# hy-vision-learning/jck-generation

Measured on AMD Instinct MI355X. Metric: images/sec (G+D step) DCGAN 64x64 bs256, higher is better.
Workload: dtype bf16; 1 GPU; DCGAN 64x64x3 synthetic, batch 256 per GPU, full G+D step incl. GP pass, RNG and Adam (BASELINE.json configs[1]); per_gpu_batch=256, global_batch=256, parallelism=dp1, dead_D_wgrad_in_G_phase=skipped (never observable: zeroed at train/dcgan_trainer.py:155)

## Files before the change

### include/jckgan.h

```cpp
#ifndef JCKGAN_H
#define JCKGAN_H
#include <stddef.h>
#include <stdint.h>
#ifdef __cplusplus
extern "C" {
#endif

#define JCK_PREC_BF16 0
#define JCK_PREC_F32 1
#define JCK_PREC_BF16X3 2

#define JCK_OK 0
#define JCK_E_ARG (-1)
#define JCK_E_HIP (-2)
#define JCK_E_WS (-3)

const char* jck_last_error(void);
const char* jck_last_launch(void);
const char* jck_launch_name(int i);
int jck_version(void);
int jck_pad_rows(int c);
int jck_pad_chan(int c);

size_t jck_packed_bytes(int prec, long long elems);
// ... 126 lines not shown
                 void* stream);
size_t jck_gp_head2_conv_ws_floats(int B);
int jck_gp_head2_conv(int prec, const void* v4, const void* a4, const float* wp, const float* prob, int B, int C, float* rs,
                      void* g_a4, float* grad, float* ws, void* stream);
size_t jck_bn2_ws_floats(int C);
int jck_bn2_vchain(int prec, const void* v, const void* y, const void* gy, const float* aux, const float* s1, const float* gamma,
                   float slope, float* ws, void* u, void* xdir, float* dgamma, long long rows, int C, void* stream);
int jck_bn2_reverse(int prec, const void* ua, const void* y, const void* xdir, const float* aux, const float* gamma,
                    const float* vsums, float slope, float* ws, void* uy, float* dgamma, float* dbeta, long long rows, int C,
                    void* stream);

int jck_adam(float* p, const float* g, float* m, float* v, long long n, double lr, double beta1, double beta2, double eps,
             int step, float grad_scale, void* stream);
int jck_adam_ema(float* p, const float* g, float* m, float* v, float* ema, long long n, double lr, double beta1, double beta2,
                 double eps, int step, float grad_scale, float ema_weight, const unsigned* skip_if, void* stream);

typedef struct jck_engine jck_engine;
int jck_engine_create(jck_engine** out, int family, int prec, int batch);
int jck_engine_create_sized(jck_engine** out, int family, int prec, int batch, int image_size);
#define JCK_ENGINE_GP_BACKWARD 1u
int jck_engine_create_ex(jck_engine** out, int family, int prec, int batch, int image_size, unsigned flags);
int jck_engine_image_size(const jck_engine*);
int jck_engine_num_tensors_of(const jck_engine*, int net);
int jck_engine_tensor_info_of(const jck_engine*, int net, int idx, char* name, int name_cap, int* kind, long long* offset,
                              long long* numel, int* shape4);
long long jck_engine_arena_numel_of(const jck_engine*, int net, int which);
void jck_engine_destroy(jck_engine*);
int jck_engine_num_tensors(int family, int net );
int jck_engine_tensor_info(int family, int net, int idx, char* name, int name_cap, int* kind, long long* offset,
                           long long* numel, int* shape4);
// ... 131 lines not shown
```

### jck-generation_amd/csrc/engine.hip

```cpp
#include <cstdlib>

#include "engine_internal.hpp"
#define JCK_BATCHED_DEFAULT 3

namespace {

constexpr long long ALIGN_F = 64;

void add_param(NetLayout& L, const char* name, int a, int b, int c, int d) {
  TensorInfo ti{name, 0, L.n_params, (long long)a * b * c * d, {a, b, c, d}};
  L.t.push_back(ti);
  L.n_params = (L.n_params + ti.numel + ALIGN_F - 1) / ALIGN_F * ALIGN_F;
}
void add_bn(NetLayout& L, const char* wn, const char* bn, const char* rm, const char* rv, int c) {
  add_param(L, wn, c, 1, 1, 1);
  add_param(L, bn, c, 1, 1, 1);
  TensorInfo m{rm, 1, L.n_bn, c, {c, 1, 1, 1}};
  L.t.push_back(m);
  L.n_bn += (c + ALIGN_F - 1) / ALIGN_F * ALIGN_F;
  TensorInfo v{rv, 2, L.n_bn, c, {c, 1, 1, 1}};
  L.t.push_back(v);
  L.n_bn += (c + ALIGN_F - 1) / ALIGN_F * ALIGN_F;
}

// ... 100 lines not shown
  e->LG = make_layout(family, 0, image_size); e->LD = make_layout(family, 1, image_size);
  e->overlap = env_on("JCK_OVERLAP");
  e->batched = getenv("JCK_BATCHED") ? atoi(getenv("JCK_BATCHED")) : JCK_BATCHED_DEFAULT;
  if (!e->overlap || batch % 8 != 0 || e->batched != 3) e->batched = 0;
  e->gp_bwd = family == 0 && (flags & JCK_ENGINE_GP_BACKWARD);
  e->carve(nullptr);
  e->wgrad_side = env_on("JCK_WGRAD_SIDE");
  e->head_side = env_on("JCK_HEAD_SIDE");
  e->ext_events = env_on("JCK_EXT_EVENTS");
  e->bn_res = env_on("JCK_BN_RES");
  e->cbuf_direct = family == 1 && env_on("JCK_CBUF_DIRECT");
  e->head_fuse = env_on("JCK_HEAD_FUSE");
  e->real_side = env_on("JCK_REAL_SIDE");
  e->fold_zero = env_on("JCK_FOLD_ZERO");
  e->fuse_tanh = env_on("JCK_FUSE_TANH");
  if (e->overlap) JCK_TRY(create_side_streams(e));
  *out = e;
  return JCK_OK;
}
extern "C" void jck_engine_destroy(jck_engine* e) {
  if (!e) return;
  if (e->overlap) destroy_side_streams(e, true);
  infer_free(e);
  delete e;
}
extern "C" int jck_engine_num_tensors(int family, int net) { return (int)make_layout(family, net).t.size(); }
static int tensor_info(const NetLayout& L, int idx, char* name, int name_cap, int* kind, long long* offset, long long* numel, int* shape4) {
  if (idx < 0 || idx >= (int)L.t.size()) JCK_FAIL(JCK_E_ARG, "index out of range");
  const TensorInfo& t = L.t[idx];
  if (name && name_cap > 0) { strncpy(name, t.name, name_cap - 1); name[name_cap - 1] = 0; }
// ... 28 lines not shown
  if (ws_bytes < e->ws_bytes) JCK_FAIL(JCK_E_WS, "workspace too small: need " + std::to_string(e->ws_bytes));
  if (((uintptr_t)workspace) % 256) JCK_FAIL(JCK_E_ARG, "workspace must be 256-byte aligned");
  e->carve(reinterpret_cast<unsigned char*>(workspace));
  {
    unsigned char* p0 = reinterpret_cast<unsigned char*>(e->d_down[0]);
    unsigned char* p1 = reinterpret_cast<unsigned char*>(e->dset[0].y[0]);
    HIPCHK(hipMemset(p0, 0, (size_t)(p1 - p0)));
  }
  HIPCHK(hipMemset(e->gsync, 0, jck_grid_sync_bytes()));
  e->gp = g_params; e->gg = g_grads; e->gm = g_m; e->gv = g_v; e->gbn = g_bn; e->gnbt = g_nbt;
  e->dp = d_params; e->dg = d_grads; e->dm = d_m; e->dv = d_v; e->dbn = d_bn; e->dnbt = d_nbt;
  e->bound = true;
  return JCK_OK;
}

static int repack_convs(jck_engine* e, int net, void* stream, const TailJobs* tail = nullptr, int tail_x = 0) {
  PackJobs jobs = {};
  int n = 0, chunk = 0;
  auto add = [&](int kind, const float* w, void* wp, long long total, int a, int b, int c) {
    PackJob& J = jobs.j[n];
    J.w = w; J.wp = wp; J.total = total; J.kind = kind; J.a = a; J.b = b; J.c = c;
    jobs.first_chunk[n] = chunk;
    chunk += (int)((total + PACK_CHUNK - 1) / PACK_CHUNK);
    ++n;
  };
  auto add_down = [&](const float* w, int Cs, int Cb, void* wp) { add(0, w, wp, (long long)Cs * Cb, Cs, Cb, ilog2(jck_pad_chan(Cb))); };
  auto add_up = [&](const float* w, int Cs, int Cb, void* wp) {
    if (Cb <= 4) add(2, w, wp, (long long)Cs * Cb, Cs, Cb, 0);
    else add(1, w, wp, (long long)Cs * Cb, Cs, Cb, jck_pad_rows(Cb));
  };
  if (net == 1) {
// ... 1 lines not shown
      const float* w = e->P(e->LD, e->dp, CWN[i]);
      add_down(w, TT.D_CS[i], TT.D_CB[i], e->d_down[i]);
      add_up(w, TT.D_CS[i], TT.D_CB[i], e->d_up[i]);
    }
    if (e->family == 0) add(4, e->P(e->LD, e->dp, CWN[TT.NS]), e->d_head_wp, TT.G_C1, TT.G_C1, 0, 0);
  } else {
    add(3, e->P(e->LG, e->gp, CWN[0]), e->g1_w, (long long)z_dim(e->family) * TT.G_C1, z_dim(e->family), TT.G_C1, z_pad(e->family));
    for (int i = 0; i < TT.NS; ++i) {
      const float* w = e->P(e->LG, e->gp, CWN[i + 1]);
      add_up(w, TT.G_CS[i], TT.G_CB[i], e->g_up[i]);
      add_down(w, TT.G_CS[i], TT.G_CB[i], e->g_down[i]);
    }
  }
  jobs.first_chunk[n] = chunk;
  jobs.n = n;
  if (net == 1) e->d_packed = true;
  if (tail) {
    const int nblk = chunk + tail_x * (tail->nl + 1);
    if (e->prec == JCK_PREC_BF16) hipLaunchKernelGGL(pack_tail_kernel<bf16_t>, dim3(nblk), dim3(256), 0, (hipStream_t)stream, jobs, chunk, *tail, tail_x);
    else hipLaunchKernelGGL(pack_tail_kernel<float>, dim3(nblk), dim3(256), 0, (hipStream_t)stream, jobs, chunk, *tail, tail_x);
  } else if (e->prec == JCK_PREC_BF16) hipLaunchKernelGGL(pack_multi_kernel<bf16_t>, dim3(chunk), dim3(256), 0, (hipStream_t)stream, jobs);
  else hipLaunchKernelGGL(pack_multi_kernel<float>, dim3(chunk), dim3(256), 0, (hipStream_t)stream, jobs);
  HIPCHK(hipGetLastError());
  return JCK_OK;
}
static int repack_linear(jck_engine* e, void* stream) {
  const float* w1 = e->P(e->LD, e->dp, "linear1.weight");
  return pack_linear_pair(e->prec, w1, L1_OUT, L1_K, L1_OUT, L1_KPAD, e->l1_w, L1_KPAD, L1_OUT, e->l1_wT, 512, 16, (hipStream_t)stream);
}
extern "C" int jck_engine_repack(jck_engine* e, int net, void* stream) {
// ... 402 lines not shown

static int refresh_adam_scalars(jck_engine* e, int step, float lr, hipStream_t st) {
  const int q = step & 1;
  JCK_TRY(jck_adam_set_step(e->hp2 + 8 * q, (double)lr, ADAM_B1, ADAM_B2, step, e->noise_seed, e->ema_w(step), st));
  e->hp_step[q] = step;
  e->hp_lr[q] = lr;
  return JCK_OK;
}
static int set_step_impl(jck_engine* e, int step, float lr, void* stream, bool zero_d);
static int adam_net(jck_engine* e, int net, long long first, long long count, float grad_scale, const float* hp, hipStream_t st,
                    float* zero_other = nullptr, float* ema = nullptr) {
  float *p = net ? e->dp : e->gp, *g = net ? e->dg : e->gg, *m = net ? e->dm : e->gm, *v = net ? e->dv : e->gv;
  return jck_adam_hp(p + first, g + first, m + first, v + first, count, ADAM_B1, ADAM_B2, ADAM_EPS, grad_scale, hp, st, zero_other,
                     zero_other ? (net ? e->LG : e->LD).n_params : 0, jck_grid_sync_error_word(e->gsync), ema);
}
static int clear_or_memset(jck_engine* e, int& clean_step, int step, hipStream_t st, void* p, size_t bytes, void* p2 = nullptr, size_t bytes2 = 0) {
  const bool clean = clean_step == step && !e->capturing;
  clean_step = -1;
  if (!clean) HIPCHK(hipMemsetAsync(p, 0, bytes, st));
  if (!clean && p2) HIPCHK(hipMemsetAsync(p2, 0, bytes2, st));
  return JCK_OK;
}
static int zero_d_grads(jck_engine* e, int step, hipStream_t st) {
  return clear_or_memset(e, e->ss.dg_clean_step, step, st, e->dg, e->LD.n_params * sizeof(float), e->family == 1 ? e->gw1p : nullptr,
                         (size_t)L1_OUT * L1_KPAD * sizeof(float));
}
static int clear_acc(jck_engine* e, int step, hipStream_t st) {
  return clear_or_memset(e, e->ss.acc_clean_step, step, st, e->acc, (size_t)8 * e->acc_ld * sizeof(float));
}

// ... 186 lines not shown

static int phase_d_step(jck_engine* e, const PhaseCtx& c) {
  if (e->ss.gp_inflight || (e->gp_bwd && e->ss.gp_done)) JCK_FAIL(JCK_E_ARG, "PHASE_D_GP must be called before PHASE_D_STEP");
  if (!e->hp_holds(c.in->step, c.in->lr) && !e->capturing) JCK_TRY(refresh_adam_scalars(e, c.in->step, c.in->lr, c.st));
  const float* hp = e->hp2 + 8 * e->parity;
  float* zg = (e->fold_zero && !e->capturing && e->LG.n_params % 4 == 0) ? e->gg : nullptr;
  if (zg) e->ss.gg_clean_step = c.in->step;
  if (e->ss.join_pending) {
    const TensorInfo* c1 = find(e->LD, CWN[0]);
    const long long cut = c1->offset + c1->numel;
    HIPCHK(hipStreamWaitEvent(c.st, e->ss.mid_recorded ? e->evWmid : e->evWdone, 0));
    JCK_TRY(adam_net(e, 1, cut, e->LD.n_params - cut, c.in->grad_scale, hp, c.st, zg));
    JCK_TRY(repack_linear(e, c.st));
    if (e->ss.mid_recorded) HIPCHK(hipStreamWaitEvent(c.st, e->evWdone, 0));
    e->ss.join_pending = e->ss.mid_recorded = false;
    JCK_TRY(adam_net(e, 1, 0, cut, c.in->grad_scale, hp, c.st));
    return repack_convs(e, 1, c.st);
  }
  JCK_TRY(adam_net(e, 1, 0, e->LD.n_params, c.in->grad_scale, hp, c.st, zg));
  return jck_engine_repack(e, 1, c.st);
}

static int phase_g_loss(jck_engine* e, const PhaseCtx& c) {
  JCK_TRY(clear_or_memset(e, e->ss.gg_clean_step, c.in->step, c.st, e->gg, e->LG.n_params * sizeof(float)));
  const bool fuse = e->head_fuse;
  JCK_TRY(d_forward(e, c.D0, e->fake, c.B, 3, c.in->drop_mask[3], c.st, !fuse));
  if (fuse && !c.cg) JCK_TRY(d_head(e, c.D0, c.B, 0.9f, 0, 2, 5, c.st, c.D0.g[TT.NS - 1]));
  else if (fuse) {
    const float tg1 = 0.9f;
    const int md1 = 0, sl1 = 2, sp1 = 5;
    JCK_TRY(cg_head_middle(e, c.B, 1, &tg1, &md1, &sl1, &sp1, c.D0.prob, c.D0.ds, c.in->drop_mask[3], c.st));
  } else JCK_TRY(d_head(e, c.D0, c.B, 0.9f, 0, 2, 5, c.st));
  XgradEpi xe = {e->fake_raw, 0.9f, e->g_raw, (c.sA && e->ext_events) ? e->evW[TT.NS - 1] : nullptr, false};
  DBackward bw;
  bw.gw = 0; bw.xgrad = true; bw.xe = e->fuse_tanh ? &xe : nullptr;
  JCK_TRY(d_backward(e, c.D0, e->fake, c.B, c.in->drop_mask[3], c.st, bw, fuse));
  return g_backward(e, c.D0.gx, c.B, c.st, c.sA, xe.fused);
}

static int phase_g_step(jck_engine* e, const PhaseCtx& c) {
  if (!e->hp_holds(c.in->step, c.in->lr) && !e->capturing) JCK_TRY(refresh_adam_scalars(e, c.in->step, c.in->lr, c.st));
  JCK_TRY(adam_net(e, 0, 0, e->LG.n_params, c.in->grad_scale, e->hp2 + 8 * e->parity, c.st, nullptr, e->gema));
  TailJobs t = {};
  for (int i = 0; i < TT.NS; ++i) {
    const int cs = TT.D_CS[i];
    t.l[i].rec = e->d_rs[i] + (size_t)e->parity * 4 * 2 * cs;
    t.l[i].rm = e->dbn + find(e->LD, RMN[i])->offset;
    t.l[i].rv = e->dbn + find(e->LD, RVN[i])->offset;
    t.l[i].nbt = (long long*)(e->dnbt + i);
    t.l[i].C = cs;
  }
  t.nl = TT.NS; t.npass = 4; t.momentum = BN_MOM; t.acc = e->acc; t.acc_ld = e->acc_ld; t.B = c.B; t.invB = 1.0f / (float)c.B; t.lambda_gp = 10.0f; t.out = e->scal_out;
  return repack_convs(e, 0, c.st, &t, cdiv(TT.G_C1, 256));
}

static int phase_begin(jck_engine* e, int phase, jck_step_inputs& loc, hipStream_t st) {
  const bool cg = e->family == 1;
  const int q = loc.step & 1;
  if (!loc.z) loc.z = e->rz[q];
  if (!loc.alpha) loc.alpha = e->ralpha[q];
  if (cg && !loc.drop_mask[0] && !loc.drop_mask[1] && !loc.drop_mask[2] && !loc.drop_mask[3])
    for (int i = 0; i < 4; ++i) loc.drop_mask[i] = e->rmask[q] + (size_t)i * e->B * L1_OUT;
  if (e->ss.join_pending && !(phase == JCK_PHASE_D_STEP || (phase == JCK_PHASE_D_GP && cg && e->ss.gp_done))) {
    HIPCHK(hipStreamWaitEvent(st, e->evWdone, 0));
    e->ss.join_pending = e->ss.mid_recorded = false;
  }
  if (cg) {
    if (!loc.labels) JCK_FAIL(JCK_E_ARG, "CGAN phases need labels");
// ... 201 lines not shown
```

### jck-generation_amd/csrc/engine_internal.hpp

```cpp
#pragma once
#include <cstring>
#include <vector>

#include "ops_internal.hpp"
#include "ew_optim.hpp"
#define JCK_INTERNAL __attribute__((visibility("hidden")))
struct jck_engine;
#define TT (e->T)

namespace jck_eng JCK_INTERNAL {

struct TensorInfo { const char* name; int kind; long long offset, numel; int shape[4]; };

struct NetLayout {
  std::vector<TensorInfo> t;
  long long n_params = 0, n_bn = 0;
};

#define JCK_MAX_STAGES 5
struct Topo {
  int S, NS, HW;
  int D_CS[JCK_MAX_STAGES], D_CB[JCK_MAX_STAGES], D_HB[JCK_MAX_STAGES];
  int G_CS[JCK_MAX_STAGES], G_CB[JCK_MAX_STAGES], G_HS[JCK_MAX_STAGES];
  int G_C1, FEAT;
// ... 80 lines not shown
  template <typename F> void for_each_side_stream(F f) { for (hipStream_t* p : {&sA, &sB, &sC}) f(*p); }
  template <typename F> void for_each_event(F f) {
    for (hipEvent_t* p : {&evWdone, &evWmid, &evHead, &evTail, &ev0, &evF, &evReal, &evGP}) f(*p);
    for (hipEvent_t& p : evW) f(p);
  }
  bool overlap = true, defer_join = true;
  bool wgrad_side = true;
  bool head_side = true;
  bool ext_events = true;
  unsigned* gsync = nullptr; bool bn_res = true;
  bool cbuf_direct = true;
  bool head_fuse = true;
  bool real_side = true;
  bool fold_zero = true;
  bool fuse_tanh = true;
  void *g_z, *g_y[JCK_MAX_STAGES], *g_a[JCK_MAX_STAGES], *g_gr[JCK_MAX_STAGES], *fake_raw, *fake, *g_raw;
  void *real_noisy, *xhat;
  BnBuf g_bn[JCK_MAX_STAGES];
  float *acc, *scal_out;
  float *acc2, *scal2;
  int acc_ld = 0;
  float *head_ws, *gp2_ws;
  float* hp2;
  unsigned long long noise_seed = 0x6a636b67616e0001ull;
  float *rz[2] = {nullptr, nullptr}, *ralpha[2] = {nullptr, nullptr}, *rmask[2] = {nullptr, nullptr};
  int hp_step[2] = {0, 0};
  float hp_lr[2] = {-1.f, -1.f};
  bool hp_holds(int step, float lr) const { return hp_step[step & 1] == step && hp_lr[step & 1] == lr; }
  bool capturing = false;
  bool gp_bwd = false;
// ... 147 lines not shown
```

### jck-generation_amd/csrc/ew_optim.hpp

```cpp
#pragma once
#include "common.hpp"
#include "philox.hpp"

struct StepRng { float* z; long long nz; float* alpha; long long nalpha; float* masks; long long nmask; float keep_p; float* zero; long long nzero;
                 float* zbig[2]; long long nzbig[2];
                 void* zpad; int zd, zp, zpad_f32; };
__device__ __forceinline__ float u01(unsigned x) { return ((float)(x >> 8) + 0.5f) * (1.0f / 16777216.0f); }
static __global__ void adam_hp_kernel(float* __restrict__ hp, float step_size, float bc2_sqrt, unsigned seed_lo, unsigned seed_hi,
                                      unsigned step, const StepRng r, float ema_w) {
  if (threadIdx.x == 0 && blockIdx.x == 0) {
    hp[0] = step_size; hp[1] = bc2_sqrt; hp[2] = ema_w;
    unsigned* w = reinterpret_cast<unsigned*>(hp + 4);
    w[0] = seed_lo; w[1] = seed_hi; w[2] = step; w[3] = 0u;
  }
  const long long q0 = (r.nz + 3) / 4, q1 = (r.nalpha + 3) / 4, q2 = (r.nmask + 3) / 4;
  for (long long i = blockIdx.x * (long long)blockDim.x + threadIdx.x; i < r.nzero; i += (long long)gridDim.x * blockDim.x) r.zero[i] = 0.f;
#pragma unroll
  for (int b = 0; b < 2; ++b)
    for (long long i = blockIdx.x * (long long)blockDim.x + threadIdx.x; i < (r.nzbig[b] >> 2); i += (long long)gridDim.x * blockDim.x)
      reinterpret_cast<f32x4*>(r.zbig[b])[i] = f32x4{0.f, 0.f, 0.f, 0.f};
  for (long long i = blockIdx.x * (long long)blockDim.x + threadIdx.x; i < q0 + q1 + q2; i += (long long)gridDim.x * blockDim.x) {
    unsigned o[4];
    if (i < q0) {
      philox4x32_10((unsigned)i, (unsigned)(i >> 32), 8u, step, seed_lo, seed_hi, o);
// ... 262 lines not shown
  if (c >= L.C) return;
  float rm = L.rm[c], rv = L.rv[c];
  for (int p = 0; p < t.npass; ++p) {
    rm = (1.f - t.momentum) * rm + t.momentum * L.rec[(long long)p * 2 * L.C + c];
    rv = (1.f - t.momentum) * rv + t.momentum * L.rec[(long long)p * 2 * L.C + L.C + c];
  }
  L.rm[c] = rm;
  L.rv[c] = rv;
}
template <typename W>
__global__ __launch_bounds__(256) void pack_tail_kernel(const PackJobs jobs, int pack_chunks, const TailJobs t, int tail_x) {
  if ((int)blockIdx.x < pack_chunks) { pack_multi_block<W>(jobs, (int)blockIdx.x); return; }
  const int q = (int)blockIdx.x - pack_chunks;
  step_tail_block(t, q % tail_x, q / tail_x);
}
```

### jck-generation_amd/csrc/ops.hip

```cpp
#include "ops_internal.hpp"
#include "ew.hpp"
#include "ew_optim.hpp"
#include "bnres.hpp"
#include "latent.hpp"

#include <cstdlib>
#include <cstring>
#include <string>

static thread_local std::string g_err;
void jck_set_error(const std::string& s) { g_err = s; }
extern "C" const char* jck_last_error(void) { return g_err.c_str(); }
#ifndef JCK_BUILD_ID
#define JCK_BUILD_ID 100
#endif
extern "C" int jck_version(void) { return JCK_BUILD_ID; }

struct KernelInfo { const char* launch; const char* label; };
#define SAME(s) {s, s}
static constexpr KernelInfo KERNELS[] = {
    SAME("igemm<bf16,128,128>"),   SAME("igemm<bf16,128,64>"),   SAME("igemm<bf16,64,128,img>"),   {nullptr, "igemm<bf16,64,128>"}, SAME("igemm<bf16,16,256>"),
    SAME("igemm<f32,128,128>"),    SAME("igemm<f32,128,64>"),    SAME("igemm<f32,64,128,img>"),    SAME("igemm<f32,64,128>"),       SAME("igemm<f32,16,256>"),
    SAME("igemm<bf16x3,128,128>"), SAME("igemm<bf16x3,128,64>"), SAME("igemm<bf16x3,64,128,img>"), SAME("igemm<bf16x3,64,128>"),    SAME("igemm<bf16x3,16,256>"),
    {"igemm_dma_persist<128,256,8>", "igemm<bf16,128,256>"}, {"igemm_dma_persist<128,128,4>", "igemm<bf16,128,128>"},
// ... 636 lines not shown
  return jck_adam_set_step(hp, 2e-4, 0.5, 0.999, step, seed, 0.f, (hipStream_t)stream, z, nz, alpha, nalpha, masks, nmask, keep_p);
}
int jck_adam_hp(float* p, const float* g, float* m, float* v, long long n, double beta1, double beta2, double eps,
                float grad_scale, const float* hp, hipStream_t st, float* zero, long long nzero, const unsigned* skip_if, float* ema) {
  const int vec = (((uintptr_t)p | (uintptr_t)g | (uintptr_t)m | (uintptr_t)v | (uintptr_t)ema) & 15) == 0;
  if (zero && (((uintptr_t)zero & 15) || (nzero & 3))) JCK_FAIL(JCK_E_ARG, "adam: the zero range must be 16-byte aligned, count % 4 == 0");
  if (ema)
    hipLaunchKernelGGL(adam_kernel<true>, dim3(ew_grid(vec ? (n + 3) / 4 : n)), dim3(256), 0, st, p, g, m, v, n, (float)(1.0 - beta1), (float)beta2,
                       (float)(1.0 - beta2), (float)eps, 0.f, 1.f, grad_scale, hp, vec, zero, zero ? nzero / 4 : 0, skip_if, ema, 1.f);
  else
    hipLaunchKernelGGL(adam_kernel<false>, dim3(ew_grid(vec ? (n + 3) / 4 : n)), dim3(256), 0, st, p, g, m, v, n, (float)(1.0 - beta1), (float)beta2,
                     (float)(1.0 - beta2), (float)eps, 0.f, 1.f, grad_scale, hp, vec, zero, zero ? nzero / 4 : 0, skip_if);
  HIPCHK(hipGetLastError());
  return JCK_OK;
}

static int launch_latent_loss(KernelId id, double bytes, int prec, const void* x, const float* target, const float* weight, const void* g_x,
                              void* g_raw, float* loss, int N, int HW, hipStream_t st) {
  ProfScope prof(id, 0.0, st, bytes);
  if (target && !weight && !g_x) {
    DISPATCH_T(prec, hipLaunchKernelGGL((latent_loss_kernel<T, true>), dim3(N), dim3(256), 0, st, (const T*)x, target, nullptr, nullptr, (T*)g_raw,
                                        loss, HW));
  } else {
    DISPATCH_T(prec, hipLaunchKernelGGL((latent_loss_kernel<T, false>), dim3(N), dim3(256), 0, st, (const T*)x, target, weight, (const T*)g_x,
                                        (T*)g_raw, loss, HW));
  }
  HIPCHK(hipGetLastError());
  return JCK_OK;
}
extern "C" int jck_latent_loss(int prec, const void* x_nhwc4, const float* target_nchw_f32, void* g_raw_out, float* loss_out, int N,
// ... 289 lines not shown
```

### jck-generation_amd/csrc/ops_internal.hpp

```cpp
#pragma once
#include <hip/hip_ext.h>

#include <algorithm>
#include <cmath>
#include <string>

#include "../../include/jckgan.h"
#include "common.hpp"

void jck_set_error(const std::string& s);

static inline bool prec_f32_storage(int prec) { return prec == JCK_PREC_F32 || prec == JCK_PREC_BF16X3; }
static inline bool is_pow2(int v) { return v > 0 && (v & (v - 1)) == 0; }
static inline unsigned ew_grid(long long n, int per_block = 256) { return (unsigned)std::max<long long>(1, std::min<long long>((n + per_block - 1) / per_block, 8192)); }

#define JCK_FAIL(code, msg)                                   \
  do {                                                        \
    jck_set_error(std::string(__func__) + ": " + (msg));     \
    return (code);                                            \
  } while (0)

#define HIPCHK(expr)                                                                                     \
  do {                                                                                                   \
    hipError_t e_ = (expr);                                                                              \
// ... 60 lines not shown
  bool on; ProfRec r;
};
bool jck_prof_is_on();

extern int g_igemm_dma_ksplit, g_bn_bwd_fuse, g_bn_res, g_wgrad_wgs, g_wgrad_ws, g_wgrad_dma;

int jck_adam_set_step(float* hp, double lr, double beta1, double beta2, int step, unsigned long long seed, float ema_w, hipStream_t st,
                      float* rz = nullptr, long long nz = 0, float* ralpha = nullptr, long long nalpha = 0, float* rmasks = nullptr,
                      long long nmask = 0, float keep_p = 0.75f, float* zero = nullptr, long long nzero = 0, float* zbig0 = nullptr,
                      long long nzbig0 = 0, float* zbig1 = nullptr, long long nzbig1 = 0, void* zpad = nullptr, int zd = 0, int zp = 0,
                      int zpad_f32 = 0);
int jck_adam_hp(float* p, const float* g, float* m, float* v, long long n, double beta1, double beta2, double eps,
                float grad_scale, const float* hp, hipStream_t st, float* zero = nullptr, long long nzero = 0,
                const unsigned* skip_if = nullptr,
                float* ema = nullptr);
const unsigned* jck_grid_sync_error_word(const void* sync_ws);
int bn_fwd_fused(int prec, const void* y, const float* stats, int slots_per_group, float count, const float* gamma, const float* beta,
                 float eps, float slope, void* a, float* aux, float* stat_out, float* running_mean, float* running_var, int64_t* nbt,
                 float momentum, long long rows_per_group, int C, int groups, long long out_row, long long out_pitch, hipStream_t stream,
                 bool* fused);
int bn_act_bwd_res_ev(int prec, const void* g_a, const void* y, const float* aux, float slope, float* sums, void* g_y, float* dgamma,
                      float* dbeta, long long rows_per_group, int C, int groups, int grad_groups, void* sync_ws, hipStream_t stream,
                      hipEvent_t done);
int conv_up_tanh_bwd_ev(int prec, const void* small_in, const void* w, const void* tanh_y, float scale, void* out, int N, int Hs, int Ws,
                        int Cs, int Cb, hipStream_t stream, hipEvent_t done, bool* fused);
int head_bwd_conv2_ev(int prec, const float* ds, const float* wp, const void* a4, int B, int B_more, int C, void* g_a4, float* grad, float* ws,
                      hipStream_t stream, hipStream_t side, hipEvent_t handover);
int gp_head2_ev(int prec, const void* ughd, const float* w2, const float* prob, int B, int K, float* rs, float* dw2, float* ws,
                hipStream_t stream, hipStream_t side, hipEvent_t handover);
int pack_linear_pair(int prec, const float* w, int N, int K, int rows0, int cols0, void* wp0, int rows1, int cols1, void* wp1, int permC,
// ... 13 lines not shown
```

### jck-generation_amd/hipgan/_lib.py

```python
import ctypes as C
import os

import torch

HERE = os.path.dirname(os.path.abspath(__file__))
LIB_PATH = os.path.join(os.path.dirname(HERE), "lib", "libjckgan_hip.so")
PREC_BF16, PREC_F32, PREC_BF16X3 = 0, 1, 2

vp, i32, i64, f32, f64, sz = C.c_void_p, C.c_int, C.c_longlong, C.c_float, C.c_double, C.c_size_t


class StepInputs(C.Structure):
    _fields_ = [("real_nchw", vp), ("noise_real", vp), ("z", vp), ("noise_fake", vp), ("alpha", vp),
                ("lr", f32), ("grad_scale", f32), ("step", i32), ("labels", vp), ("drop_mask", vp * 4),
                ("real_u8", vp), ("real_idx", vp)]


PROTOS = {
    "jck_last_error": (C.c_char_p, []),
    "jck_last_launch": (C.c_char_p, []),
    "jck_launch_name": (C.c_char_p, [i32]),
    "jck_version": (i32, []),
    "jck_pad_rows": (i32, [i32]),
    "jck_pad_chan": (i32, [i32]),
    "jck_packed_bytes": (sz, [i32, i64]),
    "jck_stats_floats": (sz, [i64, i32, i32]),
    "jck_pack_down": (i32, [i32, vp, i32, i32, vp, vp]),
    "jck_pack_up": (i32, [i32, vp, i32, i32, vp, vp]),
    "jck_pack_g1": (i32, [i32, vp, i32, i32, i32, vp, vp]),
    "jck_pack_head": (i32, [vp, i32, vp, vp]),
# ... 61 lines not shown
    "jck_sum_vec": (i32, [vp, i32, vp, vp]),
    "jck_cgan_z": (i32, [i32, vp, vp, i32, i32, i32, i32, vp, vp]),
    "jck_gp_grad": (i32, [i32, vp, vp, f32, i32, i32, vp, vp]),
    "jck_gp_head2": (i32, [i32, vp, vp, vp, i32, i32, vp, vp, vp, vp]),
    "jck_gp_head2_conv_ws_floats": (sz, [i32]),
    "jck_gp_head2_conv": (i32, [i32, vp, vp, vp, vp, i32, i32, vp, vp, vp, vp, vp]),
    "jck_bn2_ws_floats": (sz, [i32]),
    "jck_bn2_vchain": (i32, [i32, vp, vp, vp, vp, vp, vp, f32, vp, vp, vp, vp, i64, i32, vp]),
    "jck_bn2_reverse": (i32, [i32, vp, vp, vp, vp, vp, vp, f32, vp, vp, vp, vp, i64, i32, vp]),
    "jck_head_bwd": (i32, [i32, vp, vp, vp, i32, i32, vp, vp, i32, vp, vp]),
    "jck_head_unpack_grad": (i32, [vp, i32, vp, i32, vp]),
    "jck_head_bwd_conv": (i32, [i32, vp, vp, vp, i32, i32, vp, vp, vp, vp]),
    "jck_head_bwd_conv2": (i32, [i32, vp, vp, vp, i32, i32, i32, vp, vp, vp, vp]),
    "jck_adam": (i32, [vp, vp, vp, vp, i64, f64, f64, f64, f64, i32, f32, vp]),
    "jck_adam_ema": (i32, [vp, vp, vp, vp, vp, i64, f64, f64, f64, f64, i32, f32, f32, vp, vp]),
    "jck_engine_create": (i32, [C.POINTER(vp), i32, i32, i32]),
    "jck_engine_create_sized": (i32, [C.POINTER(vp), i32, i32, i32, i32]),
    "jck_engine_create_ex": (i32, [C.POINTER(vp), i32, i32, i32, i32, C.c_uint]),
    "jck_engine_image_size": (i32, [vp]),
    "jck_engine_num_tensors_of": (i32, [vp, i32]),
    "jck_engine_tensor_info_of": (i32, [vp, i32, i32, C.c_char_p, i32, C.POINTER(i32), C.POINTER(i64), C.POINTER(i64),
                                        C.POINTER(i32)]),
    "jck_engine_arena_numel_of": (i64, [vp, i32, i32]),
    "jck_engine_destroy": (None, [vp]),
    "jck_engine_num_tensors": (i32, [i32, i32]),
    "jck_engine_tensor_info": (i32, [i32, i32, i32, C.c_char_p, i32, C.POINTER(i32), C.POINTER(i64), C.POINTER(i64),
                                     C.POINTER(i32)]),
    "jck_engine_workspace_bytes": (sz, [vp]),
    "jck_engine_arena_numel": (i64, [i32, i32, i32]),
    "jck_engine_bind": (i32, [vp, vp, sz] + [vp] * 12),
# ... 127 lines not shown
```

Measured before the change: 165,700 images/sec.

## Fuse Adam update with conv weight repacking into one kernel

Adds an adam_pack kernel that applies the Adam (and EMA) update tile by tile on conv weights and writes the packed bf16/f32 conv layouts straight from LDS, so updated weights are not reread from global memory. Params outside any conv job go through a flat Adam path in the same launch, and the BN tail jobs ride along as extra blocks. This removes one launch and one full pass over the weights in the D and G step phases. In exchange the kernel uses uncoalesced tile-based Adam access and adds range bookkeeping on the host.

```diff
diff --git a/include/jckgan.h b/include/jckgan.h
--- a/include/jckgan.h
+++ b/include/jckgan.h
@@ -164,6 +164,10 @@
              int step, float grad_scale, void* stream);
 int jck_adam_ema(float* p, const float* g, float* m, float* v, float* ema, long long n, double lr, double beta1, double beta2,
                  double eps, int step, float grad_scale, float ema_weight, const unsigned* skip_if, void* stream);
+typedef struct { int kind; long long offset; void* wp; int a, b, c; } jck_pack_job;
+int jck_adam_pack(float* p, const float* g, float* m, float* v, float* ema, long long n, const jck_pack_job* jobs, int njobs,
+                  int prec, double beta1, double beta2, double eps, float grad_scale, const float* hp, float* zero,
+                  long long nzero, const unsigned* skip_if, int fused, void* stream);
 
 typedef struct jck_engine jck_engine;
 int jck_engine_create(jck_engine** out, int family, int prec, int batch);
diff --git a/jck-generation_amd/csrc/engine.hip b/jck-generation_amd/csrc/engine.hip
--- a/jck-generation_amd/csrc/engine.hip
+++ b/jck-generation_amd/csrc/engine.hip
@@ -138,6 +138,7 @@
   e->real_side = env_on("JCK_REAL_SIDE");
   e->fold_zero = env_on("JCK_FOLD_ZERO");
   e->fuse_tanh = env_on("JCK_FUSE_TANH");
+  e->adam_pack = env_on("JCK_ADAM_PACK");
   if (e->overlap) JCK_TRY(create_side_streams(e));
   *out = e;
   return JCK_OK;
@@ -196,7 +197,7 @@
   return JCK_OK;
 }
 
-static int repack_convs(jck_engine* e, int net, void* stream, const TailJobs* tail = nullptr, int tail_x = 0) {
+static PackJobs pack_jobs(jck_engine* e, int net, int* chunks) {
   PackJobs jobs = {};
   int n = 0, chunk = 0;
   auto add = [&](int kind, const float* w, void* wp, long long total, int a, int b, int c) {
@@ -228,6 +229,12 @@
   }
   jobs.first_chunk[n] = chunk;
   jobs.n = n;
+  *chunks = chunk;
+  return jobs;
+}
+static int repack_convs(jck_engine* e, int net, void* stream, const TailJobs* tail = nullptr, int tail_x = 0) {
+  int chunk = 0;
+  const PackJobs jobs = pack_jobs(e, net, &chunk);
   if (net == 1) e->d_packed = true;
   if (tail) {
     const int nblk = chunk + tail_x * (tail->nl + 1);
@@ -660,6 +667,19 @@
   return jck_adam_hp(p + first, g + first, m + first, v + first, count, ADAM_B1, ADAM_B2, ADAM_EPS, grad_scale, hp, st, zero_other,
                      zero_other ? (net ? e->LG : e->LD).n_params : 0, jck_grid_sync_error_word(e->gsync), ema);
 }
+static int adam_repack_net(jck_engine* e, int net, long long first, long long count, float grad_scale, const float* hp, hipStream_t st,
+                           float* zero_other = nullptr, float* ema = nullptr, const TailJobs* tail = nullptr, int tail_x = 0) {
+  if (!e->adam_pack) {
+    JCK_TRY(adam_net(e, net, first, count, grad_scale, hp, st, zero_other, ema));
+    return repack_convs(e, net, st, tail, tail_x);
+  }
+  int chunk = 0;
+  const PackJobs jobs = pack_jobs(e, net, &chunk);
+  if (net == 1) e->d_packed = true;
+  float *p = net ? e->dp : e->gp, *g = net ? e->dg : e->gg, *m = net ? e->dm : e->gm, *v = net ? e->dv : e->gv;
+  return jck_adam_pack_hp(p, g, m, v, (net ? e->LD : e->LG).n_params, first, count, jobs, e->prec, ADAM_B1, ADAM_B2, ADAM_EPS, grad_scale, hp, st,
+                          zero_other, zero_other ? (net ? e->LG : e->LD).n_params : 0, jck_grid_sync_error_word(e->gsync), ema, tail, tail_x);
+}
 static int clear_or_memset(jck_engine* e, int& clean_step, int step, hipStream_t st, void* p, size_t bytes, void* p2 = nullptr, size_t bytes2 = 0) {
   const bool clean = clean_step == step && !e->capturing;
   clean_step = -1;
@@ -876,11 +896,10 @@
     JCK_TRY(repack_linear(e, c.st));
     if (e->ss.mid_recorded) HIPCHK(hipStreamWaitEvent(c.st, e->evWdone, 0));
     e->ss.join_pending = e->ss.mid_recorded = false;
-    JCK_TRY(adam_net(e, 1, 0, cut, c.in->grad_scale, hp, c.st));
-    return repack_convs(e, 1, c.st);
-  }
-  JCK_TRY(adam_net(e, 1, 0, e->LD.n_params, c.in->grad_scale, hp, c.st, zg));
-  return jck_engine_repack(e, 1, c.st);
+    return adam_repack_net(e, 1, 0, cut, c.in->grad_scale, hp, c.st);
+  }
+  JCK_TRY(adam_repack_net(e, 1, 0, e->LD.n_params, c.in->grad_scale, hp, c.st, zg));
+  return c.cg ? repack_linear(e, c.st) : JCK_OK;
 }
 
 static int phase_g_loss(jck_engine* e, const PhaseCtx& c) {
@@ -902,7 +921,6 @@
 
 static int phase_g_step(jck_engine* e, const PhaseCtx& c) {
   if (!e->hp_holds(c.in->step, c.in->lr) && !e->capturing) JCK_TRY(refresh_adam_scalars(e, c.in->step, c.in->lr, c.st));
-  JCK_TRY(adam_net(e, 0, 0, e->LG.n_params, c.in->grad_scale, e->hp2 + 8 * e->parity, c.st, nullptr, e->gema));
   TailJobs t = {};
   for (int i = 0; i < TT.NS; ++i) {
     const int cs = TT.D_CS[i];
@@ -913,7 +931,7 @@
     t.l[i].C = cs;
   }
   t.nl = TT.NS; t.npass = 4; t.momentum = BN_MOM; t.acc = e->acc; t.acc_ld = e->acc_ld; t.B = c.B; t.invB = 1.0f / (float)c.B; t.lambda_gp = 10.0f; t.out = e->scal_out;
-  return repack_convs(e, 0, c.st, &t, cdiv(TT.G_C1, 256));
+  return adam_repack_net(e, 0, 0, e->LG.n_params, c.in->grad_scale, e->hp2 + 8 * e->parity, c.st, nullptr, e->gema, &t, cdiv(TT.G_C1, 256));
 }
 
 static int phase_begin(jck_engine* e, int phase, jck_step_inputs& loc, hipStream_t st) {
diff --git a/jck-generation_amd/csrc/engine_internal.hpp b/jck-generation_amd/csrc/engine_internal.hpp
--- a/jck-generation_amd/csrc/engine_internal.hpp
+++ b/jck-generation_amd/csrc/engine_internal.hpp
@@ -118,6 +118,7 @@
   bool real_side = true;
   bool fold_zero = true;
   bool fuse_tanh = true;
+  bool adam_pack = true;
   void *g_z, *g_y[JCK_MAX_STAGES], *g_a[JCK_MAX_STAGES], *g_gr[JCK_MAX_STAGES], *fake_raw, *fake, *g_raw;
   void *real_noisy, *xhat;
   BnBuf g_bn[JCK_MAX_STAGES];
diff --git a/jck-generation_amd/csrc/ew_optim.hpp b/jck-generation_amd/csrc/ew_optim.hpp
--- a/jck-generation_amd/csrc/ew_optim.hpp
+++ b/jck-generation_amd/csrc/ew_optim.hpp
@@ -300,3 +300,175 @@
   const int q = (int)blockIdx.x - pack_chunks;
   step_tail_block(t, q % tail_x, q / tail_x);
 }
+
+#define AP_TS 16
+#define AP_TB 16
+#define AP_SC 17
+#define AP_SR (AP_TB * AP_SC + 1)
+#define AP_MAX_RANGES (PACK_MAX_JOBS + 1)
+struct AdamPack {
+  float* p; const float* g; float* m; float* v; float* ema;
+  const float* hp; float* zero; const unsigned* skip_if;
+  long long nzero4, ufirst, fuse_end;
+  float w1, beta2, omb2, eps, grad_scale;
+  int vec, tiles, rest_blocks, nr;
+  int first_tile[PACK_MAX_JOBS + 1];
+  int other[PACK_MAX_JOBS];
+  int upd[PACK_MAX_JOBS];
+  long long rfirst[AP_MAX_RANGES], rcount[AP_MAX_RANGES];
+};
+__device__ __forceinline__ void adam_one_as(bool fuse_v, float& pi, float g_raw, float& m_io, float& v_io, float w1, float beta2, float omb2,
+                                            float eps, float step_size, float bc2_sqrt, float grad_scale) {
+#pragma clang fp contract(off)
+  const float gi = g_raw * grad_scale;
+  const float d = __builtin_fmaf(grad_scale, g_raw, -m_io);
+  const float mi = (w1 < 0.5f) ? __builtin_fmaf(w1, d, m_io) : __builtin_fmaf(-(1.f - w1), d, gi);
+  const float t = (omb2 * gi) * gi;
+  const float vi = fuse_v ? __builtin_fmaf(beta2, v_io, t) : v_io * beta2 + t;
+  m_io = mi;
+  v_io = vi;
+  const float denom = sqrtf(vi) / bc2_sqrt + eps;
+  pi = __builtin_fmaf(-step_size, mi / denom, pi);
+}
+__device__ __forceinline__ float ema_one_as(float e, float pn, float w) {
+#pragma clang fp contract(off)
+  const float d = pn - e;
+  return (w < 0.5f) ? __builtin_fmaf(w, d, e) : __builtin_fmaf(-(1.f - w), d, pn);
+}
+struct AdamQuad { float p[4], g[4], m[4], v[4], e[4]; };
+__device__ __forceinline__ void ap_ld4(const float* src, bool v4, float (&d)[4]) {
+  if (v4) { const f32x4 t = *reinterpret_cast<const f32x4*>(src); d[0] = t[0]; d[1] = t[1]; d[2] = t[2]; d[3] = t[3]; }
+  else { d[0] = src[0]; d[1] = src[1]; d[2] = src[2]; d[3] = src[3]; }
+}
+__device__ __forceinline__ void ap_st4(float* dst, bool v4, const float (&s)[4]) {
+  if (v4) *reinterpret_cast<f32x4*>(dst) = f32x4{s[0], s[1], s[2], s[3]};
+  else { dst[0] = s[0]; dst[1] = s[1]; dst[2] = s[2]; dst[3] = s[3]; }
+}
+template <bool EMA>
+__device__ __forceinline__ void ap_load(const AdamPack& a, long long i, bool v4, bool upd, AdamQuad& q) {
+  ap_ld4(a.p + i, v4, q.p);
+  if (upd) {
+    ap_ld4(a.g + i, v4, q.g); ap_ld4(a.m + i, v4, q.m); ap_ld4(a.v + i, v4, q.v);
+    if (EMA) ap_ld4(a.ema + i, v4, q.e);
+  }
+}
+template <bool EMA>
+__device__ __forceinline__ void ap_update_store(const AdamPack& a, long long i, bool v4, AdamQuad& q, float step_size, float bc2_sqrt, float ema_w) {
+#pragma unroll
+  for (int k = 0; k < 4; ++k) {
+    adam_one_as(i + k < a.fuse_end, q.p[k], q.g[k], q.m[k], q.v[k], a.w1, a.beta2, a.omb2, a.eps, step_size, bc2_sqrt, a.grad_scale);
+    if (EMA) q.e[k] = ema_one_as(q.e[k], q.p[k], ema_w);
+  }
+  ap_st4(a.p + i, v4, q.p); ap_st4(a.m + i, v4, q.m); ap_st4(a.v + i, v4, q.v);
+  if (EMA) ap_st4(a.ema + i, v4, q.e);
+}
+template <typename W>
+__device__ __forceinline__ void ap_emit(const PackJob& J, const float* lds, int cs0, int cb0, int ns, int nb) {
+  W* wp = reinterpret_cast<W*>(J.wp);
+  const int tid = (int)threadIdx.x;
+  switch (J.kind) {
+    case 0: {
+      const int l = tid & (AP_TB - 1);
+      if (l < nb)
+        for (int s = tid / AP_TB; s < ns * 16; s += 256 / AP_TB) {
+          const int r = s >> 4, t = s & 15;
+          stf(wp + (((long long)(cs0 + r) * 16 + t) << J.c) + cb0 + l, lds[r * AP_SR + l * AP_SC + t]);
+        }
+    } break;
+    case 1: {
+      const int l = tid & (AP_TS - 1), Cs = J.a;
+      const long long K = 4ll * Cs, per = (long long)J.c * K;
+      if (l < ns)
+        for (int s = tid / AP_TS; s < nb * 16; s += 256 / AP_TS) {
+          const int c = s >> 4, phase = (s >> 2) & 3, t = s & 3;
+          const int kh = c_up_k[phase >> 1][t >> 1], kw = c_up_k[phase & 1][t & 1];
+          stf(wp + phase * per + (long long)(cb0 + c) * K + (long long)t * Cs + cs0 + l, lds[l * AP_SR + c * AP_SC + kh * 4 + kw]);
+        }
+    } break;
+    case 2: {
+      const int l = tid & (AP_TS - 1), Cs = J.a;
+      const long long K = 9ll * Cs;
+      if (l < ns)
+        for (int s = tid / AP_TS; s < nb * 36; s += 256 / AP_TS) {
+          const int c = s / 36, q = s - c * 36, phase = q / 9, t9 = q - phase * 9;
+          const int dy = t9 / 3 - 1, dx = t9 % 3 - 1, ph = phase >> 1, pw = phase & 1;
+          const int kh = ph == 0 ? (dy == 0 ? 1 : (dy == -1 ? 3 : -1)) : (dy == 1 ? 0 : (dy == 0 ? 2 : -1));
+          const int kw = pw == 0 ? (dx == 0 ? 1 : (dx == -1 ? 3 : -1)) : (dx == 1 ? 0 : (dx == 0 ? 2 : -1));
+          if (kh >= 0 && kw >= 0) stf(wp + (long long)(phase * 4 + cb0 + c) * K + (long long)t9 * Cs + cs0 + l, lds[l * AP_SR + c * AP_SC + kh * 4 + kw]);
+        }
+    } break;
+    case 3: {
+      const int l = tid & (AP_TS - 1), Co = J.b;
+      if (l < ns)
+        for (int s = tid / AP_TS; s < nb * 16; s += 256 / AP_TS) {
+          const int c = s >> 4, t = s & 15;
+          stf(wp + ((long long)t * Co + cb0 + c) * J.c + cs0 + l, lds[l * AP_SR + c * AP_SC + t]);
+        }
+    } break;
+    default: {
+      const int l = tid & (AP_TB - 1), t = tid / AP_TB;
+      if (l < nb) reinterpret_cast<float*>(J.wp)[(long long)t * J.a + cb0 + l] = lds[l * AP_SC + t];
+    } break;
+  }
+}
+template <typename W, bool EMA>
+__global__ __launch_bounds__(256) void adam_pack_kernel(const PackJobs jobs, const AdamPack a, const TailJobs tail, int tail_x) {
+  const int bx = (int)blockIdx.x, nblk = a.tiles + a.rest_blocks;
+  if (bx >= nblk) { const int q = bx - nblk; step_tail_block(tail, q % tail_x, q / tail_x); return; }
+  __shared__ float lds[AP_TS * AP_SR];
+  const float step_size = a.hp[0], bc2_sqrt = a.hp[1], ema_w = EMA ? a.hp[2] : 1.f;
+  const bool skip = a.skip_if && *a.skip_if != 0u;
+  for (long long i = bx * 256ll + threadIdx.x; i < a.nzero4; i += nblk * 256ll) reinterpret_cast<f32x4*>(a.zero)[i] = f32x4{0.f, 0.f, 0.f, 0.f};
+  if (skip) return;
+  if (bx >= a.tiles) {
+    const long long t0 = (bx - a.tiles) * 256ll + threadIdx.x, stride = a.rest_blocks * 256ll;
+    for (int r = 0; r < a.nr; ++r) {
+      const long long first = a.rfirst[r], n = a.rcount[r];
+      const long long n4 = (a.vec && ((first - a.ufirst) & 3) == 0) ? (n >> 2) : 0;
+      for (long long i = t0; i < n4; i += stride) {
+        AdamQuad q;
+        ap_load<EMA>(a, first + 4 * i, true, true, q);
+        ap_update_store<EMA>(a, first + 4 * i, true, q, step_size, bc2_sqrt, ema_w);
+      }
+      for (long long i = first + (n4 << 2) + t0; i < first + n; i += stride) {
+        adam_one_as(i < a.fuse_end, a.p[i], a.g[i], a.m[i], a.v[i], a.w1, a.beta2, a.omb2, a.eps, step_size, bc2_sqrt, a.grad_scale);
+        if (EMA) a.ema[i] = ema_one_as(a.ema[i], a.p[i], ema_w);
+      }
+    }
+    return;
+  }
+  int ji = 0;
+  while (ji + 1 < jobs.n && bx >= a.first_tile[ji + 1]) ++ji;
+  const PackJob& J = jobs.j[ji];
+  const int Cs = J.kind == 4 ? 1 : J.a, Cb = J.kind == 4 ? J.a : J.b;
+  const int tb = (Cb + AP_TB - 1) / AP_TB, t = bx - a.first_tile[ji];
+  const int cs0 = (t / tb) * AP_TS, cb0 = (t % tb) * AP_TB;
+  const int ns = min(AP_TS, Cs - cs0), nb = min(AP_TB, Cb - cb0);
+  const long long off = J.w - a.p;
+  const bool v4 = a.vec && ((off - a.ufirst) & 3) == 0, upd = a.upd[ji] != 0;
+  const int wave = (int)threadIdx.x >> 6, c = ((int)threadIdx.x & 63) >> 2, q4 = ((int)threadIdx.x & 3) * 4;
+  static_assert(AP_TS == 8 || AP_TS == 16, "two or four passes");
+  {
+    AdamQuad q0, q1, q2, q3;
+    auto idx = [&](int r) { return off + ((long long)(cs0 + r) * Cb + cb0 + c) * 16 + q4; };
+    auto load = [&](int i, AdamQuad& q) {
+      const int r = i * 4 + wave;
+      if (r < ns && c < nb) ap_load<EMA>(a, idx(r), v4, upd, q);
+    };
+    auto update = [&](int i, AdamQuad& q) {
+      const int r = i * 4 + wave;
+      if (r < ns && c < nb) {
+        if (upd) ap_update_store<EMA>(a, idx(r), v4, q, step_size, bc2_sqrt, ema_w);
+        float* d = lds + r * AP_SR + c * AP_SC + q4;
+        d[0] = q.p[0]; d[1] = q.p[1]; d[2] = q.p[2]; d[3] = q.p[3];
+      }
+    };
+    load(0, q0); load(1, q1);
+    if (AP_TS > 8) { load(2, q2); load(3, q3); }
+    update(0, q0); update(1, q1);
+    if (AP_TS > 8) { update(2, q2); update(3, q3); }
+  }
+  __syncthreads();
+  ap_emit<W>(J, lds, cs0, cb0, ns, nb);
+  if (a.other[ji] >= 0) ap_emit<W>(jobs.j[a.other[ji]], lds, cs0, cb0, ns, nb);
+}
diff --git a/jck-generation_amd/csrc/ops.hip b/jck-generation_amd/csrc/ops.hip
--- a/jck-generation_amd/csrc/ops.hip
+++ b/jck-generation_amd/csrc/ops.hip
@@ -674,6 +674,99 @@
   HIPCHK(hipGetLastError());
   return JCK_OK;
 }
+int jck_adam_pack_hp(float* p, const float* g, float* m, float* v, long long n, long long ufirst, long long ucount, const PackJobs& jobs,
+                     int prec, double beta1, double beta2, double eps, float grad_scale, const float* hp, hipStream_t st, float* zero,
+                     long long nzero, const unsigned* skip_if, float* ema, const TailJobs* tail, int tail_x) {
+  if (!hp) JCK_FAIL(JCK_E_ARG, "adam_pack: the step scalars come from device memory (hp)");
+  if (ufirst < 0 || ucount < 0 || ufirst + ucount > n) JCK_FAIL(JCK_E_ARG, "adam_pack: the updated range leaves the arena");
+  if (jobs.n < 0 || jobs.n > PACK_MAX_JOBS) JCK_FAIL(JCK_E_ARG, "adam_pack: too many jobs");
+  if (zero && (((uintptr_t)zero & 15) || (nzero & 3))) JCK_FAIL(JCK_E_ARG, "adam: the zero range must be 16-byte aligned, count % 4 == 0");
+  if (prec != JCK_PREC_BF16 && !prec_f32_storage(prec)) JCK_FAIL(JCK_E_ARG, "bad prec");
+  AdamPack a = {};
+  a.p = p; a.g = g; a.m = m; a.v = v; a.ema = ema; a.hp = hp; a.zero = zero; a.skip_if = skip_if; a.nzero4 = zero ? nzero / 4 : 0;
+  a.w1 = (float)(1.0 - beta1); a.beta2 = (float)beta2; a.omb2 = (float)(1.0 - beta2); a.eps = (float)eps; a.grad_scale = grad_scale;
+  a.vec = (((uintptr_t)(p + ufirst) | (uintptr_t)(g + ufirst) | (uintptr_t)(m + ufirst) | (uintptr_t)(v + ufirst) | (uintptr_t)(ema ? ema + ufirst : nullptr)) & 15) == 0;
+  a.ufirst = ufirst;
+  a.fuse_end = a.vec ? ufirst + (ucount & ~3ll) : 0;
+  struct Span { long long first, count; };
+  Span done[PACK_MAX_JOBS]; int nd = 0;
+  int tiles = 0;
+  for (int j = 0; j < jobs.n; ++j) {
+    const PackJob& J = jobs.j[j];
+    a.other[j] = -1;
+    a.first_tile[j] = tiles;
+    int owner = -1;
+    for (int i = 0; i < j; ++i) if (jobs.j[i].w == J.w) { owner = i; break; }
+    if (owner >= 0) {
+      if (a.other[owner] >= 0) JCK_FAIL(JCK_E_ARG, "adam_pack: more than two layouts of one weight");
+      a.other[owner] = j;
+      continue;
+    }
+    const long long Cs = J.kind == 4 ? 1 : J.a, Cb = J.kind == 4 ? J.a : J.b, numel = Cs * Cb * 16, off = J.w - p;
+    if (Cs < 1 || Cb < 1 || J.w < p || off + numel > n) JCK_FAIL(JCK_E_ARG, "adam_pack: a job's weight lies outside the arena");
+    const bool in = off >= ufirst && off + numel <= ufirst + ucount, out = off + numel <= ufirst || off >= ufirst + ucount;
+    if (!in && !out) JCK_FAIL(JCK_E_ARG, "adam_pack: a job's weight straddles the updated range");
+    a.upd[j] = in;
+    if (in) { done[nd].first = off; done[nd].count = numel; ++nd; }
+    tiles += (int)(((Cs + AP_TS - 1) / AP_TS) * ((Cb + AP_TB - 1) / AP_TB));
+  }
+  a.first_tile[jobs.n] = tiles;
+  a.tiles = tiles;
+  std::sort(done, done + nd, [](const Span& x, const Span& y) { return x.first < y.first; });
+  long long cur = ufirst, rest = 0;
+  for (int i = 0; i <= nd; ++i) {
+    const long long stop = i < nd ? done[i].first : ufirst + ucount;
+    if (stop < cur) JCK_FAIL(JCK_E_ARG, "adam_pack: two jobs' weights overlap");
+    if (stop > cur) { a.rfirst[a.nr] = cur; a.rcount[a.nr] = stop - cur; ++a.nr; rest += stop - cur; }
+    if (i < nd) cur = done[i].first + done[i].count;
+  }
+  a.rest_blocks = (int)std::min<long long>((rest / 4 + 255) / 256, 2048);
+  if (rest > 0 && a.rest_blocks == 0) a.rest_blocks = 1;
+  if (tiles + a.rest_blocks == 0) a.rest_blocks = 1;
+  TailJobs t = {};
+  if (tail) t = *tail;
+  const int nblk = tiles + a.rest_blocks + (tail ? tail_x * (tail->nl + 1) : 0);
+  if (prec == JCK_PREC_BF16) {
+    if (ema) hipLaunchKernelGGL((adam_pack_kernel<bf16_t, true>), dim3(nblk), dim3(256), 0, st, jobs, a, t, tail_x);
+    else hipLaunchKernelGGL((adam_pack_kernel<bf16_t, false>), dim3(nblk), dim3(256), 0, st, jobs, a, t, tail_x);
+  } else {
+    if (ema) hipLaunchKernelGGL((adam_pack_kernel<float, true>), dim3(nblk), dim3(256), 0, st, jobs, a, t, tail_x);
+    else hipLaunchKernelGGL((adam_pack_kernel<float, false>), dim3(nblk), dim3(256), 0, st, jobs, a, t, tail_x);
+  }
+  HIPCHK(hipGetLastError());
+  return JCK_OK;
+}
+extern "C" int jck_adam_pack(float* p, const float* g, float* m, float* v, float* ema, long long n, const jck_pack_job* jobs, int njobs,
+                             int prec, double beta1, double beta2, double eps, float grad_scale, const float* hp, float* zero,
+                             long long nzero, const unsigned* skip_if, int fused, void* stream) {
+  if (!p || !g || !m || !v || !hp || n < 0) JCK_FAIL(JCK_E_ARG, "adam_pack: null argument");
+  if (njobs < 0 || njobs > PACK_MAX_JOBS || (njobs && !jobs)) JCK_FAIL(JCK_E_ARG, "adam_pack: 0..12 jobs");
+  if (prec != JCK_PREC_BF16 && !prec_f32_storage(prec)) JCK_FAIL(JCK_E_ARG, "bad prec");
+  PackJobs pj = {};
+  int chunk = 0;
+  for (int j = 0; j < njobs; ++j) {
+    const jck_pack_job& s = jobs[j];
+    if (s.kind < 0 || s.kind > 4 || !s.wp || s.a < 1 || (s.kind != 4 && s.b < 1)) JCK_FAIL(JCK_E_ARG, "adam_pack: bad job");
+    const long long Cs = s.kind == 4 ? 1 : s.a, Cb = s.kind == 4 ? s.a : s.b;
+    if (s.offset < 0 || s.offset + Cs * Cb * 16 > n) JCK_FAIL(JCK_E_ARG, "adam_pack: a job's weight lies outside the arena");
+    if ((s.kind == 2 && Cb > 4) || (s.kind == 3 && s.c < s.a) || (s.kind == 1 && s.c < s.b) || (s.kind == 0 && (1 << s.c) < s.b))
+      JCK_FAIL(JCK_E_ARG, "adam_pack: a job's padded size is smaller than its real one");
+    PackJob& J = pj.j[j];
+    J.w = p + s.offset; J.wp = s.wp; J.total = Cs * Cb; J.kind = s.kind; J.a = s.a; J.b = s.b; J.c = s.c;
+    pj.first_chunk[j] = chunk;
+    chunk += (int)((J.total + PACK_CHUNK - 1) / PACK_CHUNK);
+  }
+  pj.first_chunk[njobs] = chunk;
+  pj.n = njobs;
+  if (fused)
+    return jck_adam_pack_hp(p, g, m, v, n, 0, n, pj, prec, beta1, beta2, eps, grad_scale, hp, (hipStream_t)stream, zero, nzero, skip_if, ema, nullptr, 0);
+  JCK_TRY(jck_adam_hp(p, g, m, v, n, beta1, beta2, eps, grad_scale, hp, (hipStream_t)stream, zero, nzero, skip_if, ema));
+  if (!chunk) return JCK_OK;
+  if (prec == JCK_PREC_BF16) hipLaunchKernelGGL(pack_multi_kernel<bf16_t>, dim3(chunk), dim3(256), 0, (hipStream_t)stream, pj);
+  else hipLaunchKernelGGL(pack_multi_kernel<float>, dim3(chunk), dim3(256), 0, (hipStream_t)stream, pj);
+  HIPCHK(hipGetLastError());
+  return JCK_OK;
+}
 
 static int launch_latent_loss(KernelId id, double bytes, int prec, const void* x, const float* target, const float* weight, const void* g_x,
                               void* g_raw, float* loss, int N, int HW, hipStream_t st) {
diff --git a/jck-generation_amd/csrc/ops_internal.hpp b/jck-generation_amd/csrc/ops_internal.hpp
--- a/jck-generation_amd/csrc/ops_internal.hpp
+++ b/jck-generation_amd/csrc/ops_internal.hpp
@@ -98,6 +98,12 @@
                 float grad_scale, const float* hp, hipStream_t st, float* zero = nullptr, long long nzero = 0,
                 const unsigned* skip_if = nullptr,
                 float* ema = nullptr);
+struct PackJobs;
+struct TailJobs;
+int jck_adam_pack_hp(float* p, const float* g, float* m, float* v, long long n, long long ufirst, long long ucount, const PackJobs& jobs,
+                     int prec, double beta1, double beta2, double eps, float grad_scale, const float* hp, hipStream_t st,
+                     float* zero = nullptr, long long nzero = 0, const unsigned* skip_if = nullptr, float* ema = nullptr,
+                     const TailJobs* tail = nullptr, int tail_x = 0);
 const unsigned* jck_grid_sync_error_word(const void* sync_ws);
 int bn_fwd_fused(int prec, const void* y, const float* stats, int slots_per_group, float count, const float* gamma, const float* beta,
                  float eps, float slope, void* a, float* aux, float* stat_out, float* running_mean, float* running_var, int64_t* nbt,
diff --git a/jck-generation_amd/hipgan/_lib.py b/jck-generation_amd/hipgan/_lib.py
--- a/jck-generation_amd/hipgan/_lib.py
+++ b/jck-generation_amd/hipgan/_lib.py
@@ -14,6 +14,10 @@
     _fields_ = [("real_nchw", vp), ("noise_real", vp), ("z", vp), ("noise_fake", vp), ("alpha", vp),
                 ("lr", f32), ("grad_scale", f32), ("step", i32), ("labels", vp), ("drop_mask", vp * 4),
                 ("real_u8", vp), ("real_idx", vp)]
+
+
+class PackJob(C.Structure):
+    _fields_ = [("kind", i32), ("offset", i64), ("wp", vp), ("a", i32), ("b", i32), ("c", i32)]
 
 
 PROTOS = {
@@ -105,6 +109,7 @@
     "jck_head_bwd_conv2": (i32, [i32, vp, vp, vp, i32, i32, i32, vp, vp, vp, vp]),
     "jck_adam": (i32, [vp, vp, vp, vp, i64, f64, f64, f64, f64, i32, f32, vp]),
     "jck_adam_ema": (i32, [vp, vp, vp, vp, vp, i64, f64, f64, f64, f64, i32, f32, f32, vp, vp]),
+    "jck_adam_pack": (i32, [vp, vp, vp, vp, vp, i64, vp, i32, i32, f64, f64, f64, f32, vp, vp, i64, vp, i32, vp]),
     "jck_engine_create": (i32, [C.POINTER(vp), i32, i32, i32]),
     "jck_engine_create_sized": (i32, [C.POINTER(vp), i32, i32, i32, i32]),
     "jck_engine_create_ex": (i32, [C.POINTER(vp), i32, i32, i32, i32, C.c_uint]),
```

Result: no change. 167,200 images/sec (median of 6 runs) (+0.9%).
